# WoojuLee24/OA-DG

Measured on AMD Instinct MI355X. Metric: images/sec training, Faster R-CNN R50-FPN + OA-DG, 1024x2048, higher is better.
Workload: dtype bf16

## Files before the change

### include/oadg_hip.h

```cpp
#ifndef OADG_HIP_H
#define OADG_HIP_H

#include <stddef.h>
#include <stdint.h>

#ifdef __cplusplus
extern "C" {
#endif

size_t oadg_supcon_workspace_bytes(int B, int D);
int oadg_supcon_fwd(const float* feats, const int64_t* labels, int B, int D, int n_labels, int ori_size,
                    int rp_size, float temper, int min_samples, float loss_weight, void* workspace,
                    size_t workspace_bytes, float* out_loss, void* stream);
int oadg_supcon_bwd(const int64_t* labels, int B, int D, int n_labels, int ori_size, int rp_size,
                    float temper, float loss_weight, const float* grad_out, void* workspace,
                    size_t workspace_bytes, float* dfeats, void* stream);
int oadg_supcon_status(const void* workspace_host_copy);

size_t oadg_cls_loss_workspace_bytes(void);
int oadg_ce_jsd_fwd(const float* logits, const int64_t* labels, const float* weights, long R, int C,
                    int mode, float avg_factor, float loss_weight, float lambda_jsd, void* workspace,
                    size_t workspace_bytes, float* out3, void* stream);
int oadg_ce_jsd_bwd(const float* logits, const int64_t* labels, const float* weights, long R, int C,
                    int mode, float avg_factor, float loss_weight, float lambda_jsd, const float* grad_out,
// ... 107 lines not shown
    int rect[4];
    int row;
    int pad_;
    long long scratch_off;
} oadg_bbox_step;
int oadg_oamix_bbox_levels(const int* rects, const double* minvs, int n, int H, int W, int* level);
size_t oadg_oamix_bbox_plan_bytes(int n);
int oadg_oamix_bbox_plan(int kind, double severity, const long long* ib, const int* support, int n, const double* draws,
                         int n_draws, int H, int W, void* staging, size_t staging_bytes, int* level_first, int* out,
                         long long* area_sum);
int oadg_oamix_bbox_chain(uint8_t* img, int H, int W, const oadg_bbox_step* steps_dev, const int* tile_prefix_dev,
                          const int* level_first_host, int n_levels, const int* tile_prefix_host, const float* My,
                          const float* Mx, uint8_t* scratch, void* stream);
typedef struct {
    uint8_t* img;
    const oadg_bbox_step* steps_dev;
    const int* tile_prefix_dev;
    const int* level_first_host;
    const int* tile_prefix_host;
    const float* My;
    const float* Mx;
    uint8_t* scratch;
    int H, W, n_levels, pad_;
} oadg_bbox_chain;
int oadg_oamix_bbox_chain_multi(const oadg_bbox_chain* chains_host, int n, void* stream);
int oadg_oamix_compose(const uint8_t* src, uint8_t* dst, int H, int W, const oadg_region_op* ops_host,
                       const int* rects_host, int n_rects, const uint8_t* luts, const float* union_f,
                       const uint8_t* union_u8, float* acc, float acc_w, int acc_mode, void* stream);
int oadg_oamix_final(const uint8_t* img, const float* acc, int H, int W, const oadg_mix_target* targets,
                     int n_targets, const float* My, const float* Mx, double m_beta, const float* mean_host,
                     const float* stdinv_host, int to_rgb, uint8_t* out_u8, void* out_norm, int out_dtype,
                     int Hp, int Wp, void* stream);
size_t oadg_oamix_final_tiles_workspace_bytes(int H, int W, int n_targets);
int oadg_oamix_final_tiles(const uint8_t* img, const float* acc, int H, int W, const oadg_mix_target* targets,
                           int n_targets, const int* fg_rects_dev, const float* My, const float* Mx, double m_beta,
                           const float* mean_host, const float* stdinv_host, int to_rgb, uint8_t* out_u8, void* out_norm,
                           int out_dtype, int Hp, int Wp, void* workspace, size_t workspace_bytes, void* stream);
int oadg_oamix_normalize(const uint8_t* img, int H, int W, const float* mean_host, const float* stdinv_host,
                         int to_rgb, void* out, int out_dtype, int Hp, int Wp, void* stream);

int oadg_png_size(const char* path, int* height, int* width);
int oadg_png_decode_bgr(const char* path, uint8_t* out, int H, int W);

int oadg_glass_shuffle_u8(uint8_t* img, int H, int W, int C, int delta, int iters, const int32_t* dxdy);
int oadg_chamfer_l2_5x5(const uint8_t* src, int H, int W, float* dist);

int oadg_resize_bilinear_u8(const uint8_t* src, int H, int W, int C, uint8_t* dst, int Hn, int Wn, void* stream);
int oadg_flip_u8(const uint8_t* src, int H, int W, int C, uint8_t* dst, int direction, void* stream);

int oadg_conv2d_nhwc_bf16(const void* x, const void* w, const float* bias, const void* residual, void* y,
                          const void* zeros16, int N, int H, int W, int C, int K, int R, int S, int stride,
                          int pad, int dil, int relu, void* stream);

int oadg_conv2d_nhwc_bf16_variant(const void* x, const void* w, const float* bias, const void* residual, void* y,
                                  const void* zeros16, int N, int H, int W, int C, int K, int R, int S, int stride,
                                  int pad, int dil, int relu, int variant, void* stream);
int oadg_conv2d_nhwc_bf16_ex(const void* x, const void* w, const float* bias, const void* residual, void* y,
                             const void* zeros16, int N, int H, int W, int C, int K, int R, int S, int stride, int pad,
                             int dil, int relu, int variant, const void* mask, float* colsum_part,
                             const void* mask_bits, void* relu_bits_out, void* stream);
long oadg_conv2d_pixel_tiles(int N, int H, int W, int C, int K, int R, int S, int stride, int pad, int dil,
                             int variant);
int oadg_colsum_reduce(const float* part, long rows, int K, float* out, void* stream);
typedef struct oadg_colsum_job {
    const float* part;
    float* out;
    float* dgamma;
    const float* mean;
    const float* var;
    int rows, K, first_block;
    float eps;
} oadg_colsum_job;
int oadg_colsum_reduce_multi(const oadg_colsum_job* jobs_dev, int n, int total_blocks, void* stream);
int oadg_conv2d_auto_variant(int N, int H, int W, int C, int K, int R, int S, int stride, int pad, int dil);
size_t oadg_conv2d_wgrad_workspace_bytes(int N, int Ho, int Wo, int C, int K, int R, int S);
int oadg_conv2d_wgrad_variant(int N, int Ho, int Wo, int C, int K, int R, int S);
int oadg_conv2d_wgrad_nhwc_bf16(const void* x, const void* dy, float* dw, const void* zeros16, void* workspace,
                                size_t workspace_bytes, int N, int H, int W, int C, int K, int R, int S,
                                int stride, int pad, int dil, void* stream);

int oadg_conv2d_wgrad_parts_nhwc_bf16(const void* x, const void* dy, const void* zeros16, void* workspace,
                                      size_t workspace_bytes, int N, int H, int W, int C, int K, int R, int S,
                                      int stride, int pad, int dil, int* splits, void* stream);
int oadg_prep_conv_weights_bwd_parts(const float* part, int splits, const float* gbias, const float* w,
                                     const float* scale, const float* mean, const float* var, float eps, int K, int C,
                                     int R, int S, float* dw, float* dgamma, int w_krsc, void* stream);

typedef struct oadg_wgrad_job {
    const void* x;
    const void* dy;
    void* part;
    long P;
    int N, H, W, C, K, R, S, stride, pad, dil;
    int Ho, Wo, splits, chunks_per_split, first_block, blocks;
    int strip_rows, pad_;
} oadg_wgrad_job;
long oadg_conv2d_wgrad_multi_plan(oadg_wgrad_job* jobs_host, int n, int target_blocks, int* xcd_first);
int oadg_conv2d_wgrad_multi(const oadg_wgrad_job* jobs_dev, int n, int total_blocks, const int* xcd_first, const void* zeros16,
                            void* stream);
typedef struct oadg_prep_bwd_job {
    const float *part, *gbias, *w, *scale, *mean, *var;
    float *dw, *dgamma;
    float eps;
    int splits, K, C, R, S, w_krsc, first_block;
} oadg_prep_bwd_job;
int oadg_prep_conv_weights_bwd_parts_multi(const oadg_prep_bwd_job* jobs_dev, int n, int total_blocks, int max_crs,
                                           void* stream);

int oadg_conv2d_nhwc_bf16_scatter(const void* x, const void* w, const float* bias, const void* residual, void* y,
                                  const void* zeros16, int N, int H, int W, int C, int K, int R, int S, int pad, int dil,
                                  int relu, int out_h, int out_w, int OH, int OW, int osh, int osw, int oph, int opw,
                                  const void* mask, float* colsum_part, const void* mask_bits, void* stream);
int oadg_conv2d_dgrad_s2_nhwc_bf16(const void* dy, const void* wt, const void* residual, void* dx, const void* zeros16,
                                   int N, int Ho, int Wo, int K, int C, int R, int H, int W, const void* mask,
                                   float* colsum_part, const void* mask_bits, void* stream);

int oadg_prep_conv_weights(const float* w, const float* gamma, const float* beta, const float* mean,
                           const float* var, float eps, const float* bias_in, int K, int C, int R, int S, void* wf,
                           void* wt, float* bias, float* scale, int w_krsc, int wt_mode, void* stream);
typedef struct oadg_prep_desc {
    const float *w, *gamma, *beta, *mean, *var, *bias_in;
    void *wf, *wt;
    float *bias, *scale;
    float eps;
    int K, C, R, S, w_krsc, wt_mode, first_block;
} oadg_prep_desc;
int oadg_prep_conv_weights_multi_blocks(int K, int C, int R, int S);
int oadg_prep_conv_weights_multi(const oadg_prep_desc* descs, int n_layers, int total_blocks, void* stream);
int oadg_prep_conv_weights_bwd(const void* gwf, const float* gbias, const float* w, const float* scale,
                               const float* mean, const float* var, float eps, int K, int C, int R, int S, float* dw,
                               float* dgamma, int w_krsc, void* stream);

int oadg_conv1x1_n16_fwd(const void* x, const void* w16, const float* bias16, void* y, long M, int C, void* stream);
long oadg_conv1x1_n16_dgrad_rows(long M);
int oadg_conv1x1_n16_dgrad(const void* dy, const void* wt, void* dx, const void* mask_bits, float* colsum_part, long M, int C,
                           void* stream);
long oadg_conv1x1_n16_wgrad_splits(long M);
long oadg_conv1x1_n16_wgrad_rows(long M);
int oadg_conv1x1_n16_wgrad(const void* x, const void* dy, float* part, float* bias_part, const void* zeros16, long M, int C,
                           void* stream);

int oadg_stem_conv7x7s2_nhwc_bf16(const void* x, const void* wp, void* y, int N, int H, int W, void* stream);

int oadg_bias_relu_maxpool_nhwc_bf16(const void* x, const float* bias, void* out, int N, int H, int W, int C,
                                     void* stream);

size_t oadg_relu_bias_bwd_workspace_bytes(long M, int K);
int oadg_relu_bias_bwd(const void* dy, int dy_is_f32, const void* y, void* g, float* dbias, void* workspace,
                       size_t workspace_bytes, long M, int K, void* stream);

int oadg_fpn_topdown_fwd(const void* lat, const void* top, void* out, int N, int H, int W, int Ht, int Wt, int C,
                         void* stream);
int oadg_fpn_topdown_bwd(const void* g, void* dtop, int N, int H, int W, int Ht, int Wt, int C, void* stream);

size_t oadg_max_iou_assign_workspace_bytes(int B, int Gmax);
int oadg_max_iou_assign(const float* boxes, long box_stride, const unsigned char* valid, const float* gts,
                        const int* gt_counts, const int64_t* gt_labels, int B, int N, int Gmax, float pos_iou_thr,
                        float neg_iou_lo, float neg_iou_hi, float min_pos_iou, int match_low_quality,
                        void* workspace, size_t workspace_bytes, int64_t* gt_inds, float* max_overlaps,
                        int64_t* labels, int* counts, void* stream);

typedef struct oadg_select_job {
    const void* gt_inds;
    long n;
    int mode;
    int k;
// ... 110 lines not shown
```

### oa-dg_amd/_lib.py

```python
import ctypes
import os
from ctypes import (POINTER, Structure, c_char_p, c_double, c_float, c_int, c_int64, c_long, c_size_t, c_void_p)

_HERE = os.path.dirname(os.path.abspath(__file__))
LIB_PATH = os.environ.get('OADG_HIP_LIB') or os.path.join(_HERE, 'csrc', 'liboadg_hip.so')
_lib = None

vp, ci, cf, cl, cs, cd = c_void_p, c_int, c_float, c_long, c_size_t, c_double


class RpnLevel(Structure):
    _fields_ = [('deltas', c_void_p), ('sN', c_long), ('sC', c_long), ('sH', c_long), ('sW', c_long), ('anchors', c_void_p),
                ('scores', c_void_p), ('index', c_void_p), ('H', c_int), ('W', c_int), ('A', c_int), ('k', c_int),
                ('dtype', c_int), ('first', c_int)]


class RpnLossLevel(Structure):
    _fields_ = [('y', c_void_p), ('gy', c_void_p), ('sN', c_long), ('sC', c_long), ('sH', c_long), ('sW', c_long),
                ('H', c_int), ('W', c_int), ('Cy', c_int), ('first', c_long), ('pix0', c_long)]


class RoiAssignImage(Structure):
    _fields_ = [('proposals', c_void_p), ('gt_bboxes', c_void_p), ('gt_labels', c_void_p), ('stride', c_int),
                ('num_gts', c_int)]


ROI_ASSIGN_MAX_IMAGES = 32


class RoiTargetEntry(Structure):
    _fields_ = [('bboxes', c_void_p), ('gt_bboxes', c_void_p), ('gt_inds', c_void_p), ('labels', c_void_p),
                ('pos_inds', c_void_p), ('neg_inds', c_void_p), ('npos', c_int), ('nneg', c_int), ('stride', c_int),
                ('batch', c_int)]


ROI_TARGET_MAX_ENTRIES = 32


class RoiSampleImage(Structure):
    _fields_ = [('gt_inds', c_void_p), ('n', c_int)]


ROI_SAMPLE_MAX_IMAGES = 8


class RegionOp(Structure):
    _fields_ = [('kind', c_int), ('param', c_int), ('image', c_void_p), ('minv', c_double * 6)]


OP_COPY, OP_LUT_AUTOCONTRAST, OP_LUT_EQUALIZE, OP_POSTERIZE, OP_SOLARIZE, OP_IMAGE, OP_BG_WARP, OP_WARP_NEG = range(8)
OP_ENH_BRIGHTNESS, OP_ENH_COLOR, OP_ENH_CONTRAST, OP_ENH_SHARPNESS = 8, 9, 10, 11

SIGNATURES = {
    'oadg_supcon_workspace_bytes': (cs, [ci, ci]),
    'oadg_supcon_fwd': (ci, [vp, vp, ci, ci, ci, ci, ci, cf, ci, cf, vp, cs, vp, vp]),
    'oadg_supcon_bwd': (ci, [vp, ci, ci, ci, ci, ci, cf, cf, vp, vp, cs, vp, vp]),
    'oadg_supcon_status': (ci, [vp]),
    'oadg_cls_loss_workspace_bytes': (cs, []),
    'oadg_ce_jsd_fwd': (ci, [vp, vp, vp, cl, ci, ci, cf, cf, cf, vp, cs, vp, vp]),
    'oadg_ce_jsd_bwd': (ci, [vp, vp, vp, cl, ci, ci, cf, cf, cf, vp, vp, vp]),
    'oadg_roi_align_fwd': (ci, [POINTER(vp), POINTER(ci), POINTER(ci), POINTER(cf), ci, ci, ci, ci, cf,
                                vp, ci, ci, ci, ci, ci, vp, vp, vp]),
    'oadg_roi_align_bwd': (ci, [POINTER(vp), POINTER(ci), POINTER(ci), POINTER(cf), ci, ci, ci, ci, cf,
                                vp, ci, ci, ci, ci, ci, vp, vp, vp]),
    'oadg_roi_order_keys': (ci, [vp, ci, ci, ci, cf, vp, vp]),
    'oadg_roi_order': (ci, [vp, ci, ci, ci, cf, vp, vp, vp]),
    'oadg_roi_align_bwd_tiles': (ci, [POINTER(vp), POINTER(ci), POINTER(ci), POINTER(cf), ci, ci, ci, cf, vp, ci, ci, ci,
                                      ci, ci, vp, vp, vp, vp, vp]),
    'oadg_rpn_loss_workspace_bytes': (cs, []),
    'oadg_rpn_loss_fwd': (ci, [vp, ci, ci, ci, cl, ci, vp, vp, vp, vp, cf, cf, cf, cf, vp, cs, vp, vp]),
    'oadg_rpn_loss_bwd': (ci, [vp, ci, ci, ci, cl, ci, vp, vp, vp, vp, cf, cf, cf, cf, vp, vp, vp]),
    'oadg_rpn_decode': (ci, [vp, ci, ci, vp, vp, cf, vp, ci, cf, vp, vp, vp, vp]),
    'oadg_rpn_order': (ci, [vp, ci, ci, vp, vp, vp, vp, vp, vp, vp, vp]),
    'oadg_rpn_gather': (ci, [ci, ci, ci, vp, vp, vp, vp, vp, vp, vp]),
    'oadg_rpn_topk_workspace_bytes': (cs, [POINTER(ci), ci, ci, ci]),
    'oadg_rpn_topk': (ci, [POINTER(vp), POINTER(cl), POINTER(ci), ci, ci, ci, ci, POINTER(vp), POINTER(vp), vp, cs, vp]),
    'oadg_nms_workspace_bytes': (cs, [ci, ci]),
    'oadg_nms_batched': (ci, [vp, vp, ci, ci, cf, ci, vp, cs, vp, vp, vp]),
    'oadg_resize_bilinear_u8': (ci, [vp, ci, ci, ci, vp, ci, ci, vp]),
    'oadg_flip_u8': (ci, [vp, ci, ci, ci, vp, ci, vp]),
    'oadg_conv2d_nhwc_bf16': (ci, [vp, vp, vp, vp, vp, vp] + [ci] * 11 + [vp]),
    'oadg_conv2d_auto_variant': (ci, [ci] * 10),
    'oadg_conv2d_nhwc_bf16_ex': (ci, [vp, vp, vp, vp, vp, vp] + [ci] * 12 + [vp, vp, vp, vp, vp]),
    'oadg_conv2d_pixel_tiles': (cl, [ci] * 11),
    'oadg_colsum_reduce': (ci, [vp, cl, ci, vp, vp]),
    'oadg_conv2d_nhwc_bf16_variant': (ci, [vp, vp, vp, vp, vp, vp] + [ci] * 12 + [vp]),
    'oadg_conv2d_wgrad_workspace_bytes': (cs, [ci] * 7),
    'oadg_conv2d_wgrad_variant': (ci, [ci] * 7),
    'oadg_conv2d_wgrad_nhwc_bf16': (ci, [vp, vp, vp, vp, vp, cs] + [ci] * 10 + [vp]),
    'oadg_conv2d_wgrad_parts_nhwc_bf16': (ci, [vp, vp, vp, vp, cs] + [ci] * 10 + [POINTER(ci), vp]),
    'oadg_prep_conv_weights_bwd_parts': (ci, [vp, ci, vp, vp, vp, vp, vp, cf, ci, ci, ci, ci, vp, vp, ci, vp]),
    'oadg_prep_conv_weights': (ci, [vp, vp, vp, vp, vp, cf, vp, ci, ci, ci, ci, vp, vp, vp, vp, ci, ci, vp]),
    'oadg_prep_conv_weights_multi': (ci, [vp, ci, ci, vp]),
    'oadg_prep_conv_weights_multi_blocks': (ci, [ci, ci, ci, ci]),
    'oadg_conv2d_nhwc_bf16_scatter': (ci, [vp, vp, vp, vp, vp, vp] + [ci] * 18 + [vp, vp, vp, vp]),
    'oadg_conv2d_dgrad_s2_nhwc_bf16': (ci, [vp, vp, vp, vp, vp, ci, ci, ci, ci, ci, ci, ci, ci, vp, vp, vp, vp]),
    'oadg_prep_conv_weights_bwd': (ci, [vp, vp, vp, vp, vp, vp, cf, ci, ci, ci, ci, vp, vp, ci, vp]),
    'oadg_relu_bias_bwd_workspace_bytes': (ctypes.c_size_t, [cl, ci]),
    'oadg_relu_bias_bwd': (ci, [vp, ci, vp, vp, vp, vp, ctypes.c_size_t, cl, ci, vp]),
    'oadg_stem_conv7x7s2_nhwc_bf16': (ci, [vp, vp, vp, ci, ci, ci, vp]),
    'oadg_bias_relu_maxpool_nhwc_bf16': (ci, [vp, vp, vp, ci, ci, ci, ci, vp]),
    'oadg_fpn_topdown_fwd': (ci, [vp, vp, vp, ci, ci, ci, ci, ci, ci, vp]),
    'oadg_fpn_topdown_bwd': (ci, [vp, vp, ci, ci, ci, ci, ci, ci, vp]),
    'oadg_max_iou_assign_workspace_bytes': (ctypes.c_size_t, [ci, ci]),
    'oadg_max_iou_assign': (ci, [vp, cl, vp, vp, vp, vp, ci, ci, ci, cf, cf, cf, cf, ci, vp, ctypes.c_size_t, vp, vp, vp,
                                 vp, vp]),
    'oadg_sample_select_workspace_bytes': (ctypes.c_size_t, [ci, cl]),
    'oadg_sample_select': (ci, [vp, ci, cl, ci, vp, vp, vp, ctypes.c_size_t, vp]),
    'oadg_anchor_targets': (ci, [vp, vp, vp, vp, vp, vp, ci, ci, ci, ci, c_int64, cf, vp, vp, vp, vp, vp, vp, vp]),
    'oadg_colsum_reduce_multi': (ci, [vp, ci, ci, vp]),
    'oadg_conv1x1_n16_fwd': (ci, [vp, vp, vp, vp, cl, ci, vp]),
    'oadg_conv1x1_n16_dgrad_rows': (cl, [cl]),
    'oadg_conv1x1_n16_dgrad': (ci, [vp, vp, vp, vp, vp, cl, ci, vp]),
    'oadg_bottleneck_frozen_256': (ci, [vp, vp, vp, vp, vp, vp, vp, vp, ci, ci, ci, vp]),
    'oadg_bottleneck_frozen_first_64': (ci, [vp, vp, vp, vp, vp, vp, vp, vp, vp, vp, ci, ci, ci, vp]),
    'oadg_conv1x1_n16_wgrad_splits': (cl, [cl]),
    'oadg_conv1x1_n16_wgrad_rows': (cl, [cl]),
    'oadg_conv1x1_n16_wgrad': (ci, [vp, vp, vp, vp, vp, cl, ci, vp]),
    'oadg_conv2d_wgrad_multi_plan': (ctypes.c_long, [vp, ci, ci, vp]),
    'oadg_conv2d_wgrad_multi': (ci, [vp, ci, ci, vp, vp, vp]),
    'oadg_prep_conv_weights_bwd_parts_multi': (ci, [vp, ci, ci, ci, vp]),
    'oadg_sgd_blocks': (ctypes.c_longlong, [ctypes.c_longlong]),
    'oadg_sgd_step_multi': (ci, [vp, ci, ctypes.c_longlong, cf, cf, cf, vp]),
    'oadg_fc_weight_permute': (ci, [vp, vp, ci, ci, ci, ci, vp]),
    'oadg_parse_losses': (ci, [vp, vp, ci, ci, ctypes.c_uint, vp, vp, vp]),
    'oadg_roi_reg_acc_fwd': (ci, [vp, ci, vp, ci, vp, vp, vp, ci, ci, ci, ci, ci, cf, cf, cf, vp, vp]),
    'oadg_roi_reg_bwd': (ci, [vp, ci, vp, vp, vp, ci, ci, ci, ci, cf, cf, cf, vp, vp, vp]),
    'oadg_roi_assign_add_gt': (ci, [vp, ci, ci, ci, cf, cf, cf, cf, ci, vp, vp, vp, vp, vp, vp, vp, vp, vp, ctypes.c_size_t,
                                    vp, vp]),
    'oadg_roi_targets': (ci, [vp, ci, ci, c_int64, cf, vp, vp, vp, vp, vp, vp, vp, vp, vp]),
    'oadg_roi_targets_dev': (ci, [vp, ci, ci, ci, vp, c_int64, cf, vp, vp, vp, vp, vp, vp, vp, vp, vp]),
    'oadg_roi_sample_max_rows': (ci, []),
    'oadg_roi_sample_device': (ci, [vp, ci, ci, ci, cf, vp, vp, vp, vp, vp, vp]),
    'oadg_conv2d_f32': (ci, [vp, vp, vp, vp, vp, ci, ci, ci, ci, ci, ci, ci, ci, ci, ci, ci, ci, ci, vp]),
    'oadg_conv2d_wgrad_f32_splits': (ci, [ci, ci, ci, ci, ci, ci, ci]),
    'oadg_conv2d_wgrad_f32': (ci, [vp, vp, vp, vp, cs, ci, ci, ci, ci, ci, ci, ci, ci, ci, ci, vp]),
    'oadg_host_randperm_prefix': (ci, [vp, POINTER(ci), POINTER(ctypes.c_uint64), c_int64, c_int64, vp]),
    'oadg_np_random_bboxes': (ci, [vp, ci, ci, ci, vp, ci, cd, cd, cd, cd, ci, cd, cd, vp]),
    'oadg_oamix_box_profiles': (ci, [vp, vp, ci, ci, ci, ci, vp, vp, vp]),
    'oadg_oamix_fg_union': (ci, [vp, vp, ci, ci, ci, vp, vp, vp]),
    'oadg_oamix_fg_union_rects': (ci, [vp, vp, vp, ci, ci, ci, vp, vp, vp]),
    'oadg_oamix_saliency_workspace_bytes': (cs, [ci]),
    'oadg_oamix_saliency': (ci, [vp, ci, ci, vp, ci, ci, vp, vp, cs, vp]),
    'oadg_oamix_saliency_batch': (ci, [vp, ctypes.c_longlong, vp, ci, ci, vp, ci, ci, vp, vp, ctypes.c_size_t, vp]),
    'oadg_oamix_hist': (ci, [vp, cl, vp, vp]),
    'oadg_oamix_luts': (ci, [vp, vp, vp]),
    'oadg_oamix_gray_sum': (ci, [vp, cl, vp, vp]),
    'oadg_oamix_bbox_step': (ci, [vp, ci, ci, POINTER(cd), ci, ci, ci, ci, vp, vp, vp, vp]),
    'oadg_oamix_bbox_levels': (ci, [POINTER(ci), POINTER(cd), ci, ci, ci, POINTER(ci)]),
    'oadg_oamix_bbox_plan_bytes': (cs, [ci]),
    'oadg_oamix_bbox_plan': (ci, [ci, cd, vp, vp, ci, vp, ci, ci, ci, vp, cs, vp, vp, vp]),
    'oadg_oamix_bbox_chain': (ci, [vp, ci, ci, vp, vp, POINTER(ci), ci, POINTER(ci), vp, vp, vp, vp]),
    'oadg_oamix_bbox_chain_multi': (ci, [vp, ci, vp]),
    'oadg_png_size': (ci, [c_char_p, POINTER(ci), POINTER(ci)]),
    'oadg_png_decode_bgr': (ci, [c_char_p, vp, ci, ci]),
    'oadg_glass_shuffle_u8': (ci, [vp, ci, ci, ci, ci, ci, vp]),
    'oadg_chamfer_l2_5x5': (ci, [vp, ci, ci, vp]),
    'oadg_oamix_compose': (ci, [vp, vp, ci, ci, POINTER(RegionOp), POINTER(ci), ci, vp, vp, vp, vp, cf, ci, vp]),
    'oadg_oamix_final': (ci, [vp, vp, ci, ci, vp, ci, vp, vp, cd, POINTER(cf), POINTER(cf), ci, vp, vp, ci, ci,
                              ci, vp]),
    'oadg_oamix_final_tiles_workspace_bytes': (ctypes.c_size_t, [ci, ci, ci]),
    'oadg_oamix_final_tiles': (ci, [vp, vp, ci, ci, vp, ci, vp, vp, vp, cd, POINTER(cf), POINTER(cf), ci, vp, vp, ci, ci,
                                    ci, vp, ctypes.c_size_t, vp]),
    'oadg_oamix_normalize': (ci, [vp, ci, ci, POINTER(cf), POINTER(cf), ci, vp, ci, ci, ci, vp]),
}


class HipLibraryMissing(RuntimeError):
    pass


def lib():
    global _lib
# ... 35 lines not shown
```

### oa-dg_amd/csrc/conv_mfma.hip

```cpp
#include <algorithm>
#include <vector>
#include "common.h"
#include <type_traits>
#include <stdlib.h>
#include "oadg_hip.h"

namespace {

constexpr int BM = 128, BN = 128, BK = 64;

struct ConvArgs {
    const unsigned short* x;
    const unsigned short* w;
    const float* bias;
    const unsigned short* res;
    unsigned short* y;
    const unsigned short* zeros;
    const unsigned short* mask;
    const unsigned char* bits_in;
    unsigned char* bits_out;
    float* colsum;
    int N, H, W, C, K, R, S, Ho, Wo, stride, pad, dil, relu;
    long M;
    int scatter, OH, OW, osh, osw, oph, opw;
// ... 1465 lines not shown

    for (int t = 0; t < nk; ++t) {
        const int buf = t & 1;
        read_x(0, buf);
        read_x(1, buf);
        read_dy(0, buf);
        stage_x(1, s1, buf ^ 1);
        stage_dy(1, s1, buf ^ 1);
        OADG_WMFMA32(0, 0);
        read_dy(1, buf);
        stage_dy(0, s2, buf);
        stage_x(0, s2, buf);
        asm volatile("s_waitcnt vmcnt(4)" ::: "memory");
        OADG_WMFMA32(1, 1);
        s1 = s2;
        advance(s2);
    }
#undef OADG_WMFMA32
    if (wr == 0) asm volatile("s_barrier" ::: "memory");
    asm volatile("s_waitcnt vmcnt(0)" ::: "memory");

    float* out = a.part + (size_t)split * a.K * RS * a.C;
    const int fr = lane & 15, cq = lane >> 4;
#pragma unroll
    for (int xh = 0; xh < 2; ++xh)
#pragma unroll
        for (int jt = 0; jt < 2; ++jt) {
            const int c = c0 + xh * 128 + wc * 32 + jt * 16 + 4 * cq;
#pragma unroll
            for (int dh = 0; dh < 2; ++dh)
#pragma unroll
                for (int it = 0; it < 4; ++it) {
                    const int k = k0 + dh * 128 + wr * 64 + it * 16 + fr;
                    *reinterpret_cast<f32x4v*>(out + ((size_t)k * RS + rs) * a.C + c) = acc[xh][jt][dh][it];
                }
        }
}

__global__ __launch_bounds__(512) void conv_wgrad256_kernel(WgradArgs a) {
    extern __shared__ __attribute__((aligned(16))) unsigned char smem[];
    const int combos = (a.K / 256) * (a.C / 256) * a.R * a.S;
    const long bid = blockIdx.x;
    int split, combo;
    if (a.splits % 8 == 0) {
        const long xcd = bid & 7, j = bid >> 3;
        combo = (int)(j % combos);
        split = (int)((j / combos) * 8 + xcd);
    } else {
        const long total = (long)a.splits * combos, per = (total + 7) >> 3;
        const long xcd = bid & 7, slot = bid >> 3, w = xcd * per + slot;
        if (slot >= per || w >= total) return;
        combo = (int)(w % combos);
        split = (int)(w / combos);
    }
    wgrad256_tile(a, split, combo, smem);
}

struct XcdSlices {
    int first[9];
};

__global__ __launch_bounds__(512) void conv_wgrad256_multi_kernel(const oadg_wgrad_job* __restrict__ jobs, int n_jobs,
                                                                  XcdSlices xs, const unsigned short* zeros) {
    extern __shared__ __attribute__((aligned(16))) unsigned char smem[];
    const int xcd = blockIdx.x & 7, slot = blockIdx.x >> 3, w = xs.first[xcd] + slot;
    if (w >= xs.first[xcd + 1]) return;
    int lo = 0, hi = n_jobs - 1;
    while (lo < hi) {
        const int mid = (lo + hi + 1) >> 1;
        if (jobs[mid].first_block <= w) lo = mid; else hi = mid - 1;
    }
    const oadg_wgrad_job& jb = jobs[__builtin_amdgcn_readfirstlane(lo)];
    WgradArgs a;
    a.x = (const unsigned short*)jb.x; a.dy = (const unsigned short*)jb.dy; a.part = (float*)jb.part; a.zeros = zeros;
    a.N = jb.N; a.H = jb.H; a.W = jb.W; a.C = jb.C; a.K = jb.K; a.R = jb.R; a.S = jb.S; a.Ho = jb.Ho; a.Wo = jb.Wo;
    a.stride = jb.stride; a.pad = jb.pad; a.dil = jb.dil; a.splits = jb.splits; a.chunks_per_split = jb.chunks_per_split;
    a.strip_rows = jb.strip_rows;
    a.P = jb.P;
    const int local = w - jb.first_block;
    const int combos = (a.K / 256) * (a.C / 256) * a.R * a.S;
    wgrad256_tile(a, local / combos, local % combos, smem);
}

__global__ void wgrad_reduce_kernel(const float* __restrict__ part, int splits, long n, float* __restrict__ dw) {
    const long i = (long)blockIdx.x * blockDim.x + threadIdx.x;
    if (i >= n) return;
    float s = 0.f;
    for (int k = 0; k < splits; ++k) s += part[(size_t)k * n + i];
    dw[i] = s;
}

long wgrad256_splits(long P, int K, int C, int RS) {
    const long tiles = (long)(K / 256) * (C / 256) * RS;
    long s = 256 / tiles;
    if (s < 1) s = 1;
    return s;
}
bool wgrad_use256(long P, int K, int C, int RS) {
    if (K % 256 != 0 || C % 256 != 0) return false;
    const long nchunks = (P + WP - 1) / WP;
    return nchunks / wgrad256_splits(P, K, C, RS) >= 8;
}
int wgrad_stages(int RS) { return RS > 1 ? 1 : 2; }

int wgrad_strip(int N, int Ho, int Wo, int RS, int& splits, int& chunks_per_split) {
    const long rows = (long)N * Ho;
    if (RS <= 1 || Wo % WP != 0 || rows < splits || splits < 1) return 0;
    const long per = (rows + splits - 1) / splits;
    splits = (int)((rows + per - 1) / per);
    chunks_per_split = (int)(per * (Wo / WP));
    return (int)per;
}

int wgrad_splits(long P, int K, int C, int RS) {
    if (wgrad_use256(P, K, C, RS)) return (int)wgrad256_splits(P, K, C, RS);
    const long tiles = (long)(K / 128) * (C / 128) * RS;
    const long nchunks = (P + WP - 1) / WP;
    const long target = 512;
    long s = (target + tiles - 1) / tiles;
    if (s > nchunks / 4) s = nchunks / 4;
    if (s >= 8) s = (s + 7) / 8 * 8;
    if (s < 1) s = 1;
    if (s > 256) s = 256;
    return (int)s;
}

}

extern "C" size_t oadg_conv2d_wgrad_workspace_bytes(int N, int Ho, int Wo, int C, int K, int R, int S) {
    if (C % 128 || K % 128) return 0;
    const int sp = wgrad_splits((long)N * Ho * Wo, K, C, R * S);
    return (size_t)sp * K * R * S * C * sizeof(float);
}

extern "C" int oadg_conv2d_wgrad_variant(int N, int Ho, int Wo, int C, int K, int R, int S) {
    if (C % 128 || K % 128) return 0;
    if (wgrad_use256((long)N * Ho * Wo, K, C, R * S)) return 256;
    return wgrad_stages(R * S);
}

namespace {
int wgrad_launch(const void* x, const void* dy, float* dw, const void* zeros16, void* workspace,
                 size_t workspace_bytes, int N, int H, int W, int C, int K, int R, int S, int stride, int pad, int dil,
                 int* splits_out, void* stream) {
    if (!x || !dy || !zeros16 || !workspace) return OADG_EARG;
    if (C % 128 != 0 || K % 128 != 0 || N < 1 || R < 1 || S < 1) return OADG_EARG;
    if ((double)N * H * W * C >= 4294967296.0) return OADG_EARG;
    WgradArgs a;
    a.x = (const unsigned short*)x; a.dy = (const unsigned short*)dy; a.part = (float*)workspace;
    a.zeros = (const unsigned short*)zeros16;
    a.N = N; a.H = H; a.W = W; a.C = C; a.K = K; a.R = R; a.S = S; a.stride = stride; a.pad = pad; a.dil = dil;
    a.Ho = (H + 2 * pad - dil * (R - 1) - 1) / stride + 1;
    a.Wo = (W + 2 * pad - dil * (S - 1) - 1) / stride + 1;
    a.P = (long)N * a.Ho * a.Wo;
    a.splits = wgrad_splits(a.P, K, C, R * S);
    const long nchunks = (a.P + WP - 1) / WP;
    a.chunks_per_split = (int)((nchunks + a.splits - 1) / a.splits);
    const size_t need = (size_t)a.splits * K * R * S * C * sizeof(float);
    if (workspace_bytes < need) return OADG_ESIZE;
    hipStream_t st = (hipStream_t)stream;
    a.strip_rows = 0;
    if (wgrad_use256(a.P, K, C, R * S)) {
        a.strip_rows = wgrad_strip(N, a.Ho, a.Wo, R * S, a.splits, a.chunks_per_split);
        static bool attr_set = false;
        if (!attr_set) {
            hipError_t e = hipFuncSetAttribute((const void*)conv_wgrad256_kernel,
                                               hipFuncAttributeMaxDynamicSharedMemorySize, 2 * BUF_BYTES);
            if (e != hipSuccess) return (int)e;
            attr_set = true;
        }
        long blocks = (long)a.splits * (K / 256) * (C / 256) * R * S;
        if (a.splits % 8 != 0) blocks = ((blocks + 7) / 8) * 8;
        hipLaunchKernelGGL(conv_wgrad256_kernel, dim3((unsigned)blocks), dim3(512), 2 * BUF_BYTES, st, a);
    } else {
        const long blocks = (long)a.splits * (K / 128) * (C / 128) * R * S;
        if (wgrad_stages(R * S) == 2)
            hipLaunchKernelGGL(conv_wgrad_kernel<2>, dim3((unsigned)blocks), dim3(256), 2 * WSTAGE, st, a);
        else
            hipLaunchKernelGGL(conv_wgrad_kernel<1>, dim3((unsigned)blocks), dim3(256), WSTAGE, st, a);
    }
    OADG_LAUNCH_CHECK();
    if (splits_out) {
        *splits_out = a.splits;
        return OADG_OK;
    }
    const long n = (long)K * R * S * C;
    hipLaunchKernelGGL(wgrad_reduce_kernel, dim3((unsigned)((n + 255) / 256)), dim3(256), 0, st,
                       (const float*)workspace, a.splits, n, dw);
    OADG_LAUNCH_CHECK();
    return OADG_OK;
}
}

extern "C" int oadg_conv2d_wgrad_nhwc_bf16(const void* x, const void* dy, float* dw, const void* zeros16,
                                           void* workspace, size_t workspace_bytes, int N, int H, int W, int C,
                                           int K, int R, int S, int stride, int pad, int dil, void* stream) {
    if (!dw) return OADG_EARG;
    return wgrad_launch(x, dy, dw, zeros16, workspace, workspace_bytes, N, H, W, C, K, R, S, stride, pad, dil, nullptr,
                        stream);
}

extern "C" int oadg_conv2d_wgrad_parts_nhwc_bf16(const void* x, const void* dy, const void* zeros16, void* workspace,
                                                 size_t workspace_bytes, int N, int H, int W, int C, int K, int R,
                                                 int S, int stride, int pad, int dil, int* splits, void* stream) {
    if (!splits) return OADG_EARG;
    return wgrad_launch(x, dy, nullptr, zeros16, workspace, workspace_bytes, N, H, W, C, K, R, S, stride, pad, dil,
                        splits, stream);
}

extern "C" long oadg_conv2d_wgrad_multi_plan(oadg_wgrad_job* jobs, int n, int target_blocks, int* xcd_first) {
    if (!jobs || n < 1 || target_blocks < 1) return -(long)OADG_EARG;
    double work = 0.0;
    for (int i = 0; i < n; ++i) {
        oadg_wgrad_job& j = jobs[i];
        if (j.N < 1 || j.H < 1 || j.W < 1 || j.R < 1 || j.S < 1 || j.stride < 1 || j.dil < 1 || j.pad < 0) return -(long)OADG_EARG;
        if (j.K % 256 != 0 || j.C % 256 != 0 || j.K < 256 || j.C < 256) return -(long)OADG_EARG;
        if ((double)j.N * j.H * j.W * j.C >= 4294967296.0) return -(long)OADG_EARG;
        j.Ho = (j.H + 2 * j.pad - j.dil * (j.R - 1) - 1) / j.stride + 1;
        j.Wo = (j.W + 2 * j.pad - j.dil * (j.S - 1) - 1) / j.stride + 1;
        if (j.Ho < 1 || j.Wo < 1) return -(long)OADG_EARG;
        j.P = (long)j.N * j.Ho * j.Wo;
        const long tiles = (long)(j.K / 256) * (j.C / 256) * j.R * j.S, nchunks = (j.P + WP - 1) / WP;
        work += (double)tiles * (double)nchunks;
    }
    auto assign = [&](long target, int* sp_out) -> long {
        const double per = work / (double)target;
        long total = 0;
        for (int i = 0; i < n; ++i) {
            const oadg_wgrad_job& j = jobs[i];
            const long nchunks = (j.P + WP - 1) / WP;
            long sp = per > 0.0 ? (long)((double)nchunks / per) : 1;
            if (sp < 1) sp = 1;
            if (sp > nchunks) sp = nchunks;
            sp_out[i] = (int)sp;
            total += (long)(j.K / 256) * (j.C / 256) * j.R * j.S * sp;
        }
        while (total > target) {
            int best = -1;
            double shortest = 1e300;
            for (int i = 0; i < n; ++i) {
                const oadg_wgrad_job& j = jobs[i];
                if (sp_out[i] <= 1) continue;
                const double len = (double)((j.P + WP - 1) / WP) / sp_out[i];
                if (len < shortest) { shortest = len; best = i; }
            }
            if (best < 0) break;
            sp_out[best] -= 1;
            total -= (long)(jobs[best].K / 256) * (jobs[best].C / 256) * jobs[best].R * jobs[best].S;
        }
        for (;;) {
            int best = -1;
            double longest = 0.0;
            for (int i = 0; i < n; ++i) {
                const oadg_wgrad_job& j = jobs[i];
                const long tiles = (long)(j.K / 256) * (j.C / 256) * j.R * j.S, nchunks = (j.P + WP - 1) / WP;
                if (sp_out[i] >= nchunks || total + tiles > target) continue;
                const double len = (double)nchunks / sp_out[i];
                if (len > longest) { longest = len; best = i; }
            }
            if (best < 0) break;
            sp_out[best] += 1;
            total += (long)(jobs[best].K / 256) * (jobs[best].C / 256) * jobs[best].R * jobs[best].S;
        }
        return total;
    };
    const int cus_per_xcd = target_blocks >= 8 ? target_blocks / 8 : 1;
    auto slices = [cus_per_xcd](const std::vector<double>& len, long* fx) -> double {
        const long cnt = (long)len.size();
        auto fill = [&](double limit, long* out, bool even) -> bool {
            long w = 0;
            double left = 0.0;
            for (double v : len) left += v;
            std::vector<double> cu((size_t)cus_per_xcd);
            for (int x = 0; x < 8; ++x) {
                out[x] = w;
                std::fill(cu.begin(), cu.end(), 0.0);
                const double share = left / (8 - x);
                double mine = 0.0;
                while (w < cnt) {
                    if (even && mine >= share) break;
                    size_t m = 0;
                    for (size_t u = 1; u < cu.size(); ++u)
                        if (cu[u] < cu[m]) m = u;
                    if (cu[m] + len[(size_t)w] > limit) break;
                    cu[m] += len[(size_t)w];
                    mine += len[(size_t)w++];
                }
                left -= mine;
            }
            out[8] = w;
// ... 430 lines not shown
```

Before: 143.0.

## Add tap-row wgrad kernel reusing x rows across 3 horizontal taps

Adds a weight-gradient kernel for 3-wide, stride-1 convolutions in which each block computes one filter row (all S=3 taps) for a 256x128 K/C tile. One staged x strip with halo feeds all three taps, cutting global loads and LDS traffic compared with the per-tap tiles. It uses transposed LDS reads and a double-buffered pipeline. By default it replaces the existing 256-tile path whenever the shape qualifies, with its own split count, which can enlarge the workspace and changes how work is spread across XCDs.

Result: no change. 143.6 (median of 4 runs) (+0.4%).

```diff
diff --git a/include/oadg_hip.h b/include/oadg_hip.h
--- a/include/oadg_hip.h
+++ b/include/oadg_hip.h
@@ -213,6 +213,10 @@
 int oadg_conv2d_wgrad_parts_nhwc_bf16(const void* x, const void* dy, const void* zeros16, void* workspace,
                                       size_t workspace_bytes, int N, int H, int W, int C, int K, int R, int S,
                                       int stride, int pad, int dil, int* splits, void* stream);
+int oadg_conv2d_wgrad_parts_variant_nhwc_bf16(const void* x, const void* dy, const void* zeros16, void* workspace,
+                                              size_t workspace_bytes, int N, int H, int W, int C, int K, int R, int S,
+                                              int stride, int pad, int dil, int form, int splits_req, int* splits,
+                                              void* stream);
 int oadg_prep_conv_weights_bwd_parts(const float* part, int splits, const float* gbias, const float* w,
                                      const float* scale, const float* mean, const float* var, float eps, int K, int C,
                                      int R, int S, float* dw, float* dgamma, int w_krsc, void* stream);
diff --git a/oa-dg_amd/_lib.py b/oa-dg_amd/_lib.py
--- a/oa-dg_amd/_lib.py
+++ b/oa-dg_amd/_lib.py
@@ -89,6 +89,7 @@
     'oadg_conv2d_wgrad_variant': (ci, [ci] * 7),
     'oadg_conv2d_wgrad_nhwc_bf16': (ci, [vp, vp, vp, vp, vp, cs] + [ci] * 10 + [vp]),
     'oadg_conv2d_wgrad_parts_nhwc_bf16': (ci, [vp, vp, vp, vp, cs] + [ci] * 10 + [POINTER(ci), vp]),
+    'oadg_conv2d_wgrad_parts_variant_nhwc_bf16': (ci, [vp, vp, vp, vp, cs] + [ci] * 12 + [POINTER(ci), vp]),
     'oadg_prep_conv_weights_bwd_parts': (ci, [vp, ci, vp, vp, vp, vp, vp, cf, ci, ci, ci, ci, vp, vp, ci, vp]),
     'oadg_prep_conv_weights': (ci, [vp, vp, vp, vp, vp, cf, vp, ci, ci, ci, ci, vp, vp, vp, vp, ci, ci, vp]),
     'oadg_prep_conv_weights_multi': (ci, [vp, ci, ci, vp]),
diff --git a/oa-dg_amd/csrc/conv_mfma.hip b/oa-dg_amd/csrc/conv_mfma.hip
--- a/oa-dg_amd/csrc/conv_mfma.hip
+++ b/oa-dg_amd/csrc/conv_mfma.hip
@@ -1571,6 +1571,226 @@
     wgrad256_tile(a, local / combos, local % combos, smem);
 }
 
+constexpr int TR_D = 16384;
+constexpr int TR_X_OFF = 2 * TR_D;
+constexpr int TR_X_ROWS = 64 + 32;
+constexpr int TR_BUF = 65536;
+constexpr int TR_LDS = TR_BUF + TR_X_OFF + TR_X_ROWS * 256;
+static_assert(TR_X_OFF + TR_X_ROWS * 256 <= TR_BUF, "tap-row buffer overflows its stride");
+static_assert(TR_LDS <= 160 * 1024, "tap-row LDS");
+
+__device__ __forceinline__ int tr_sw(int row) { return ((row & 3) << 2) | (((row >> 3) & 1) << 1); }
+
+template <int OFF>
+__device__ __forceinline__ void tr_read(bf16x8& f, int half, unsigned addr) {
+    v4s v;
+    asm volatile("ds_read_b64_tr_b16 %0, %1 offset:%2" : "=v"(v) : "v"(addr), "i"(OFF));
+    f[half * 4 + 0] = v[0]; f[half * 4 + 1] = v[1]; f[half * 4 + 2] = v[2]; f[half * 4 + 3] = v[3];
+}
+__device__ __forceinline__ void tr_fence(bf16x8& f) { asm volatile("" : "+v"(f)); }
+
+template <int DIL>
+__device__ __forceinline__ void wgrad256_taprow_tile(const WgradArgs& a, const int split, const int combo,
+                                                     unsigned char* smem) {
+    const int tid = threadIdx.x, lane = tid & 63;
+    const int wave = __builtin_amdgcn_readfirstlane(tid >> 6);
+    const int wr = wave >> 2, wc = wave & 3;
+    const int kt_n = a.K / 256, ct_n = a.C / 128, RS = a.R * a.S;
+    const int ct = combo % ct_n;
+    const int kt = (combo / ct_n) % kt_n;
+    const int r = combo / (ct_n * kt_n);
+    const int k0 = kt * 256, c0 = ct * 128;
+    const int spr = a.Wo / WP;
+    const long rows_total = (long)a.N * a.Ho;
+    const long row0 = (long)split * a.strip_rows;
+    const long row1 = row0 + a.strip_rows < rows_total ? row0 + a.strip_rows : rows_total;
+    const int nrows = row1 > row0 ? (int)(row1 - row0) : 0;
+    const int nk = nrows * spr;
+
+    const int lrow = tid >> 4;
+    const int lslot = (tid & 15) ^ tr_sw(lrow);
+    const long dH = (long)a.W * a.C, dN = (long)a.H * a.W * a.C;
+    const long chunk_dy = (long)WP * a.K;
+    const uintptr_t dyb = (uintptr_t)(a.dy + (size_t)lrow * a.K + k0 + lslot * 8);
+    const uintptr_t dy_piece = (uintptr_t)32 * a.K * 2;
+    const int xcb = c0 + lslot * 8;
+    const int halo = wave == 0 && lrow < 2 * DIL;
+
+    struct TrState {
+        int t, k, sidx, ho, hi;
+        long ch, xrow;
+    };
+    auto init_state = [&](TrState& st) {
+        st.ch = row0 * spr + st.sidx;
+        st.ho = (int)(row0 % a.Ho);
+        const long n = row0 / a.Ho;
+        st.hi = st.ho - a.pad + r * DIL;
+        st.xrow = n * dN + (long)st.hi * dH;
+    };
+    auto advance = [&](TrState& st) {
+        st.t++;
+        if (++st.k >= nrows) {
+            st.k = 0;
+            ++st.sidx;
+            if (st.t < nk) init_state(st);
+        } else {
+            st.ch += spr;
+            ++st.ho; ++st.hi;
+            st.xrow += dH;
+            if (st.ho >= a.Ho) {
+                st.ho -= a.Ho; st.hi -= a.Ho;
+                st.xrow += dN - (long)a.Ho * dH;
+            }
+        }
+    };
+    auto stage_dy = [&](int h, const TrState& st, int buf) {
+        unsigned char* dst = smem + buf * TR_BUF + h * TR_D + wave * 1024;
+        const bool live = st.t < nk;
+        const uintptr_t src = dyb + (uintptr_t)(st.ch * chunk_dy + h * 128) * 2;
+        glds16((const void*)(live ? src : (uintptr_t)a.zeros), dst);
+        glds16((const void*)(live ? src + dy_piece : (uintptr_t)a.zeros), dst + 8192);
+    };
+    auto stage_x = [&](const TrState& st, int buf) {
+        unsigned char* dst = smem + buf * TR_BUF + TR_X_OFF + wave * 1024;
+        const bool rok = st.t < nk && (unsigned)st.hi < (unsigned)a.H;
+        const int wi = st.sidx * WP - a.pad + lrow;
+        const unsigned short* src = a.x + st.xrow + (long)wi * a.C + xcb;
+        const bool ok0 = rok && (unsigned)wi < (unsigned)a.W;
+        const bool ok1 = rok && (unsigned)(wi + 32) < (unsigned)a.W;
+        const bool ok2 = rok && halo && (unsigned)(wi + 64) < (unsigned)a.W;
+        glds16(ok0 ? (const void*)src : (const void*)a.zeros, dst);
+        glds16(ok1 ? (const void*)(src + 32 * a.C) : (const void*)a.zeros, dst + 8192);
+        glds16(ok2 ? (const void*)(src + 64 * a.C) : (const void*)a.zeros, dst + 16384);
+    };
+
+    f32x4v acc[3][2][2][4];
+#pragma unroll
+    for (int x0 = 0; x0 < 3; ++x0)
+#pragma unroll
+        for (int x1 = 0; x1 < 2; ++x1)
+#pragma unroll
+            for (int x2 = 0; x2 < 2; ++x2)
+#pragma unroll
+                for (int x3 = 0; x3 < 4; ++x3) acc[x0][x1][x2][x3] = f32x4v{0.f, 0.f, 0.f, 0.f};
+
+    const int frow = (lane >> 4) * 8 + ((lane & 15) >> 2);
+    int dyoff0, xct0;
+    {
+        const int c4 = (lane & 3) * 4;
+        const int chd = wr * 64 + c4, chx = wc * 32 + c4;
+        dyoff0 = frow * 256 + (((chd >> 3) ^ tr_sw(frow)) << 4) + (chd & 7) * 2;
+        xct0 = ((chx >> 3) << 4) + (chx & 7) * 2;
+    }
+    bf16x8 df[4], xf[3][2];
+    const unsigned lds0 = (unsigned)(uintptr_t)smem;
+    auto read_dy = [&](auto H, auto KS, int bo) {
+        int d0 = dyoff0;
+        asm volatile("" : "+v"(d0));
+#pragma unroll
+        for (int it = 0; it < 4; ++it) {
+            const unsigned addr = lds0 + ((d0 ^ (it << 5)) | bo);
+            tr_read<decltype(H)::value * TR_D + decltype(KS)::value * 8192>(df[it], 0, addr);
+            tr_read<decltype(H)::value * TR_D + decltype(KS)::value * 8192 + 1024>(df[it], 1, addr);
+        }
+    };
+    auto read_x = [&](auto KS, int bo) {
+        int rw = frow, xc = xct0;
+        asm volatile("" : "+v"(rw), "+v"(xc));
+#pragma unroll
+        for (int s = 0; s < 3; ++s)
+#pragma unroll
+            for (int u = 0; u < 2; ++u) {
+                const int xr = rw + s * DIL + u * 4;
+                const int rt = ((TR_X_OFF + xr * 256) | (tr_sw(xr) << 4)) | bo;
+#pragma unroll
+                for (int jt = 0; jt < 2; ++jt)
+                    tr_read<decltype(KS)::value * 8192>(xf[s][jt], u, lds0 + (rt ^ xc ^ (jt << 5)));
+            }
+    };
+#define OADG_TMFMA24(DH)                                                                                     \
+    do {                                                                                                     \
+        asm volatile("s_waitcnt lgkmcnt(0)" ::: "memory");                                                   \
+        asm volatile("s_barrier" ::: "memory");                                                              \
+        _Pragma("unroll") for (int it = 0; it < 4; ++it) tr_fence(df[it]);                                   \
+        _Pragma("unroll") for (int s = 0; s < 3; ++s) { tr_fence(xf[s][0]); tr_fence(xf[s][1]); }            \
+        __builtin_amdgcn_sched_barrier(0);                                                                   \
+        __builtin_amdgcn_s_setprio(1);                                                                       \
+        _Pragma("unroll") for (int s = 0; s < 3; ++s)                                                        \
+            _Pragma("unroll") for (int jt = 0; jt < 2; ++jt)                                                 \
+                _Pragma("unroll") for (int it = 0; it < 4; ++it)                                             \
+                    acc[s][jt][DH][it] = __builtin_amdgcn_mfma_f32_16x16x32_bf16(xf[s][jt], df[it],           \
+                                                                                 acc[s][jt][DH][it], 0, 0, 0); \
+        __builtin_amdgcn_s_setprio(0);                                                                       \
+        __builtin_amdgcn_sched_barrier(0);                                                                   \
+        asm volatile("s_barrier" ::: "memory");                                                              \
+    } while (0)
+
+    TrState s1, s2;
+    s1.t = s1.k = s1.sidx = 0;
+    init_state(s1);
+    stage_dy(0, s1, 0);
+    stage_dy(1, s1, 0);
+    stage_x(s1, 0);
+    advance(s1);
+    stage_dy(0, s1, 1);
+    s2 = s1;
+    advance(s2);
+    asm volatile("s_waitcnt vmcnt(2)" ::: "memory");
+    asm volatile("s_barrier" ::: "memory");
+    if (wr == 1) asm volatile("s_barrier" ::: "memory");
+
+    for (int t = 0; t < nk; ++t) {
+        const int buf = t & 1, bo = buf * TR_BUF, nb = buf ^ 1;
+        using I0 = std::integral_constant<int, 0>;
+        using I1 = std::integral_constant<int, 1>;
+        read_x(I0{}, bo);
+        read_dy(I0{}, I0{}, bo);
+        stage_dy(1, s1, nb);
+        OADG_TMFMA24(0);
+        read_dy(I1{}, I0{}, bo);
+        stage_x(s1, nb);
+        OADG_TMFMA24(1);
+        read_x(I1{}, bo);
+        read_dy(I0{}, I1{}, bo);
+        OADG_TMFMA24(0);
+        read_dy(I1{}, I1{}, bo);
+        stage_dy(0, s2, buf);
+        asm volatile("s_waitcnt vmcnt(2)" ::: "memory");
+        OADG_TMFMA24(1);
+        s1 = s2;
+        advance(s2);
+    }
+#undef OADG_TMFMA24
+    if (wr == 0) asm volatile("s_barrier" ::: "memory");
+    asm volatile("s_waitcnt vmcnt(0)" ::: "memory");
+
+    float* out = a.part + (size_t)split * a.K * RS * a.C;
+    const int fr = lane & 15, cq = lane >> 4;
+#pragma unroll
+    for (int s = 0; s < 3; ++s)
+#pragma unroll
+        for (int jt = 0; jt < 2; ++jt) {
+            const int c = c0 + wc * 32 + jt * 16 + 4 * cq;
+#pragma unroll
+            for (int dh = 0; dh < 2; ++dh)
+#pragma unroll
+                for (int it = 0; it < 4; ++it) {
+                    const int k = k0 + dh * 128 + wr * 64 + it * 16 + fr;
+                    *reinterpret_cast<f32x4v*>(out + ((size_t)k * RS + r * a.S + s) * a.C + c) = acc[s][jt][dh][it];
+                }
+        }
+}
+
+template <int DIL>
+__global__ __launch_bounds__(512) void conv_wgrad256_taprow_kernel(WgradArgs a) {
+    extern __shared__ __attribute__((aligned(16))) unsigned char smem[];
+    const int combos = (a.K / 256) * (a.C / 128) * a.R;
+    const long total = (long)a.splits * combos, per = (total + 7) >> 3;
+    const long xcd = blockIdx.x & 7, slot = blockIdx.x >> 3, w = xcd * per + slot;
+    if (slot >= per || w >= total) return;
+    wgrad256_taprow_tile<DIL>(a, (int)(w / combos), (int)(w % combos), smem);
+}
+
 __global__ void wgrad_reduce_kernel(const float* __restrict__ part, int splits, long n, float* __restrict__ dw) {
     const long i = (long)blockIdx.x * blockDim.x + threadIdx.x;
     if (i >= n) return;
@@ -1599,6 +1819,19 @@
     splits = (int)((rows + per - 1) / per);
     chunks_per_split = (int)(per * (Wo / WP));
     return (int)per;
+}
+
+long wgrad_taprow_combos(int K, int C, int R) { return (long)(K / 256) * (C / 128) * R; }
+long wgrad_taprow_splits(int K, int C, int R) {
+    const long s = 256 / wgrad_taprow_combos(K, C, R);
+    return s < 1 ? 1 : s;
+}
+bool wgrad_taprow_shape(long P, int N, int Ho, int Wo, int K, int C, int R, int S) {
+    if (S != 3 || Wo % WP != 0 || !wgrad_use256(P, K, C, R * S)) return false;
+    return (long)N * Ho >= wgrad_taprow_splits(K, C, R);
+}
+bool wgrad_taprow_ok(long P, int N, int Ho, int Wo, int K, int C, int R, int S, int stride, int dil) {
+    return stride == 1 && dil >= 1 && dil <= 2 && wgrad_taprow_shape(P, N, Ho, Wo, K, C, R, S);
 }
 
 int wgrad_splits(long P, int K, int C, int RS) {
@@ -1618,7 +1851,9 @@
 
 extern "C" size_t oadg_conv2d_wgrad_workspace_bytes(int N, int Ho, int Wo, int C, int K, int R, int S) {
     if (C % 128 || K % 128) return 0;
-    const int sp = wgrad_splits((long)N * Ho * Wo, K, C, R * S);
+    long sp = wgrad_splits((long)N * Ho * Wo, K, C, R * S);
+    if (wgrad_taprow_shape((long)N * Ho * Wo, N, Ho, Wo, K, C, R, S) && wgrad_taprow_splits(K, C, R) > sp)
+        sp = wgrad_taprow_splits(K, C, R);
     return (size_t)sp * K * R * S * C * sizeof(float);
 }
 
@@ -1631,7 +1866,7 @@
 namespace {
 int wgrad_launch(const void* x, const void* dy, float* dw, const void* zeros16, void* workspace,
                  size_t workspace_bytes, int N, int H, int W, int C, int K, int R, int S, int stride, int pad, int dil,
-                 int* splits_out, void* stream) {
+                 int* splits_out, void* stream, int form = 0, int splits_req = 0) {
     if (!x || !dy || !zeros16 || !workspace) return OADG_EARG;
     if (C % 128 != 0 || K % 128 != 0 || N < 1 || R < 1 || S < 1) return OADG_EARG;
     if ((double)N * H * W * C >= 4294967296.0) return OADG_EARG;
@@ -1642,15 +1877,36 @@
     a.Ho = (H + 2 * pad - dil * (R - 1) - 1) / stride + 1;
     a.Wo = (W + 2 * pad - dil * (S - 1) - 1) / stride + 1;
     a.P = (long)N * a.Ho * a.Wo;
-    a.splits = wgrad_splits(a.P, K, C, R * S);
+    if (form != 0 && form != 1 && form != 3) return OADG_EARG;
+    const bool use256 = wgrad_use256(a.P, K, C, R * S);
+    const bool taprow_ok = wgrad_taprow_ok(a.P, N, a.Ho, a.Wo, K, C, R, S, stride, dil);
+    if ((form == 1 && !use256) || (form == 3 && !taprow_ok) || (splits_req > 0 && !use256)) return OADG_EARG;
+    const bool taprow = form == 3 || (form == 0 && taprow_ok);
+    a.splits = taprow ? (int)wgrad_taprow_splits(K, C, R) : wgrad_splits(a.P, K, C, R * S);
+    if (splits_req > 0) a.splits = splits_req;
     const long nchunks = (a.P + WP - 1) / WP;
     a.chunks_per_split = (int)((nchunks + a.splits - 1) / a.splits);
+    a.strip_rows = 0;
+    if (use256) a.strip_rows = wgrad_strip(N, a.Ho, a.Wo, R * S, a.splits, a.chunks_per_split);
+    if (taprow && a.strip_rows <= 0) return OADG_EARG;
     const size_t need = (size_t)a.splits * K * R * S * C * sizeof(float);
     if (workspace_bytes < need) return OADG_ESIZE;
     hipStream_t st = (hipStream_t)stream;
-    a.strip_rows = 0;
-    if (wgrad_use256(a.P, K, C, R * S)) {
-        a.strip_rows = wgrad_strip(N, a.Ho, a.Wo, R * S, a.splits, a.chunks_per_split);
+    if (taprow) {
+        static bool attr_set = false;
+        if (!attr_set) {
+            for (const void* f : {(const void*)conv_wgrad256_taprow_kernel<1>, (const void*)conv_wgrad256_taprow_kernel<2>}) {
+                hipError_t e = hipFuncSetAttribute(f, hipFuncAttributeMaxDynamicSharedMemorySize, TR_LDS);
+                if (e != hipSuccess) return (int)e;
+            }
+            attr_set = true;
+        }
+        const long blocks = ((long)a.splits * wgrad_taprow_combos(K, C, R) + 7) / 8 * 8;
+        if (dil == 1)
+            hipLaunchKernelGGL(conv_wgrad256_taprow_kernel<1>, dim3((unsigned)blocks), dim3(512), TR_LDS, st, a);
+        else
+            hipLaunchKernelGGL(conv_wgrad256_taprow_kernel<2>, dim3((unsigned)blocks), dim3(512), TR_LDS, st, a);
+    } else if (use256) {
         static bool attr_set = false;
         if (!attr_set) {
             hipError_t e = hipFuncSetAttribute((const void*)conv_wgrad256_kernel,
@@ -1695,6 +1951,15 @@
     if (!splits) return OADG_EARG;
     return wgrad_launch(x, dy, nullptr, zeros16, workspace, workspace_bytes, N, H, W, C, K, R, S, stride, pad, dil,
                         splits, stream);
+}
+
+extern "C" int oadg_conv2d_wgrad_parts_variant_nhwc_bf16(const void* x, const void* dy, const void* zeros16, void* workspace,
+                                                         size_t workspace_bytes, int N, int H, int W, int C, int K, int R,
+                                                         int S, int stride, int pad, int dil, int form, int splits_req,
+                                                         int* splits, void* stream) {
+    if (!splits || splits_req < 0) return OADG_EARG;
+    return wgrad_launch(x, dy, nullptr, zeros16, workspace, workspace_bytes, N, H, W, C, K, R, S, stride, pad, dil,
+                        splits, stream, form, splits_req);
 }
 
 extern "C" long oadg_conv2d_wgrad_multi_plan(oadg_wgrad_job* jobs, int n, int target_blocks, int* xcd_first) {
```
